# PROBIC/mSWEEP

Hardware: AMD Instinct MI355X
Metric: EM iters/sec + reads×groups cells/sec, 10M reads × 5k groups (higher is better)
Workload: dtype f64

## Files before the change

include/msweep_core.h:

```cpp
#ifndef MSWEEP_CORE_H
#define MSWEEP_CORE_H

#include <stddef.h>
#include <stdint.h>

#ifdef __cplusplus
extern "C" {
#endif

typedef struct msw_core *msw_handle;

enum { MSW_ALGO_RCG = 0, MSW_ALGO_EM = 1 };
enum { MSW_PREC_DOUBLE = 0, MSW_PREC_FLOAT = 1 };

int msw_core_create(int device, msw_handle *out);
void msw_core_destroy(msw_handle h);
const char *msw_last_error(msw_handle h);
const char *msw_core_version(void);


int msw_core_set_dense_logl(msw_handle h, const double *L, size_t n_groups, size_t n_ecs,
                            size_t ld);

int msw_core_set_csr(msw_handle h, const uint64_t *rowptr, const uint32_t *grp,
// ... 7 lines not shown
                              const uint64_t *ec_counts, double q, double e,
                              double zero_inflation, size_t min_hits,
                              size_t *n_groups_out, uint8_t *mask_out, double *logc_out);

int msw_core_get_dense_logl(msw_handle h, double *L_out, size_t ld);
int msw_core_layout_hash(msw_handle h, uint64_t *hash_out);
int msw_core_shape(msw_handle h, size_t *n_groups, size_t *n_ecs, size_t *nnz);
typedef struct msw_layout_info {
  int32_t record_bytes;
  int32_t index_records;
  int32_t groups_in_lds;
  int32_t table_in_lds;
  int32_t passB_mode;
  uint32_t slot_entries;
  uint32_t slot_entries_in_lds;
  uint32_t n_slices, n_long_ecs;
  uint64_t rows;
  uint64_t rows_from_memory;
  uint32_t slices_by_lanes[7];
  uint32_t max_rows;
  int32_t bank_scheduled;
  int32_t passB_reg_cells;
  uint64_t rows_over_8;
} msw_layout_info;
int msw_core_layout_info(msw_handle h, msw_layout_info *out);
int msw_core_set_pack_schedule(msw_handle h, int enabled);

enum { MSW_OPT_CHECK_EVERY = 0, MSW_OPT_INIT_BOUND = 1, MSW_OPT_EM_PRIOR = 2, MSW_OPT_EM_STOP = 3 };
int msw_core_set_option(msw_handle h, int option, double value);
int msw_core_get_option(msw_handle h, int option, double *value);

int msw_core_solve(msw_handle h, const double *logc, const double *alpha0, double tol,
                   size_t max_iters, int algo, int prec, double *theta_out,
                   size_t *iters_out, double *bound_out);

int msw_core_prepare(msw_handle h, const double *logc, const double *alpha0);
int msw_core_run(msw_handle h, double tol, size_t max_iters, int algo, int prec,
                 double *theta_out, size_t *iters_out, double *bound_out);

int msw_core_gamma(msw_handle h, double *gamma_out, size_t ld);

int msw_core_gamma_block(msw_handle h, size_t ec_begin, size_t ec_end, double *gamma_out, size_t ld);

int msw_core_bin_reads(msw_handle h, const uint64_t *ec_rptr, const uint32_t *ec_reads, size_t n_ecs,
                       const uint32_t *targets, const double *thresholds, size_t n_targets, uint64_t *bin_ptr,
                       uint32_t *reads_out, double *log_thr_out);
// ... 108 lines not shown
```

msweep_amd/core.py:

```python
import ctypes as C
import os

import numpy as np

_HERE = os.path.dirname(os.path.abspath(__file__))
LIB_PATH = os.environ.get("MSWEEP_CORE_LIB") or os.path.join(_HERE, "libmsweep_core.so")

ALGO_RCG, ALGO_EM = 0, 1
PREC_DOUBLE, PREC_FLOAT = 0, 1
TEXT_PROBS, TEXT_LOGL, TEXT_BITSEQ = 0, 1, 2
OPT_CHECK_EVERY, OPT_INIT_BOUND, OPT_EM_PRIOR, OPT_EM_STOP = 0, 1, 2, 3
_OPTS = {"check_every": OPT_CHECK_EVERY, "init_bound": OPT_INIT_BOUND, "em_prior": OPT_EM_PRIOR, "em_stop": OPT_EM_STOP}

EXPORTS = [
    "msw_core_create", "msw_core_destroy", "msw_last_error", "msw_core_version",
    "msw_core_set_dense_logl", "msw_core_set_csr", "msw_core_build_likelihood",
    "msw_core_get_dense_logl", "msw_core_layout_hash", "msw_core_shape", "msw_alignment_read",
    "msw_alignment_shape", "msw_alignment_export", "msw_alignment_view", "msw_alignment_destroy", "msw_alignment_last_error",
    "msw_alignment_read_device", "msw_core_build_likelihood_aln", "msw_core_trim", "msw_alignment_on_device", "msw_core_solve", "msw_core_prepare", "msw_core_run",
    "msw_core_gamma",
    "msw_core_trace", "msw_core_set_trace_theta", "msw_core_bootstrap",
    "msw_core_resample_counts", "msw_core_set_profiling", "msw_core_last_timing",
    "msw_core_set_fixed_iters", "msw_core_hbm_stream_rates", "msw_comm_unique_id", "msw_comm_create_rccl", "msw_comm_create_local",
    "msw_comm_destroy", "msw_core_set_comm", "msw_comm_last_error", "msw_core_bootstrap_dist",
# ... 2 lines not shown
    "msw_core_set_option", "msw_core_get_option", "msw_core_bin_reads", "msw_core_bin_reads_aln",
    "msw_core_text_block", "msw_core_format_g6", "msw_core_last_text_timing",
    "msw_core_gzip_begin", "msw_core_text_block_gzip", "msw_core_gzip_append", "msw_core_gzip_end", "msw_core_last_gzip_timing",
]


class MswError(RuntimeError):
    """Non-zero return from the C ABI (mirrors the std::runtime_error the C++ shim throws)."""


class Timing(C.Structure):
    _fields_ = [("solve_ms", C.c_double), ("passA_ms", C.c_double), ("passB_ms", C.c_double),
                ("passA_launches", C.c_uint64), ("passB_launches", C.c_uint64), ("iters", C.c_uint64),
                ("bytes_passA", C.c_uint64), ("bytes_passB", C.c_uint64), ("collective_ms", C.c_double),
                ("collectives", C.c_uint64), ("em_float_kernels", C.c_uint64)]


class LayoutInfo(C.Structure):
    _fields_ = [("record_bytes", C.c_int32), ("index_records", C.c_int32), ("groups_in_lds", C.c_int32),
                ("table_in_lds", C.c_int32), ("passB_mode", C.c_int32), ("slot_entries", C.c_uint32),
                ("slot_entries_in_lds", C.c_uint32), ("n_slices", C.c_uint32), ("n_long_ecs", C.c_uint32),
                ("rows", C.c_uint64), ("rows_from_memory", C.c_uint64), ("slices_by_lanes", C.c_uint32 * 7),
                ("max_rows", C.c_uint32), ("bank_scheduled", C.c_int32), ("passB_reg_cells", C.c_int32),
                ("rows_over_8", C.c_uint64)]


class BootstrapTiming(C.Structure):
    _fields_ = [("table_ms", C.c_double), ("solve_ms", C.c_double), ("gather_ms", C.c_double),
                ("replicates", C.c_uint64), ("iterations", C.c_uint64), ("table_reused", C.c_uint64)]


_lib = None


def source_hash():
    import hashlib
    csrc = os.path.join(_HERE, "csrc")
    h = hashlib.sha256()
    files = sorted(os.path.join(csrc, f) for f in os.listdir(csrc) if f.endswith((".hip", ".hpp", ".inc", ".h")))
    for f in files + [os.path.join(os.path.dirname(_HERE), "include", "msweep_core.h")]:
        h.update(os.path.basename(f).encode() + b"\0")
        h.update(open(f, "rb").read())
    return h.hexdigest()[:16]


def _check_fresh(L):
    if os.environ.get("MSWEEP_CORE_LIB"):
# ... 615 lines not shown
```

msweep_amd/csrc/common.hpp:

```cpp
#pragma once
#include <hip/hip_runtime.h>

#include <cstdint>
#include <cstdio>
#include <stdexcept>
#include <string>
#include <vector>

namespace msw {

constexpr int kWave = 64;
#ifndef MSW_PASS_THREADS_A
#define MSW_PASS_THREADS_A 1024
#endif
#ifndef MSW_PASS_THREADS_B
#define MSW_PASS_THREADS_B 768
#endif
#ifndef MSW_PASS_THREADS_B8
#define MSW_PASS_THREADS_B8 1024
#endif
constexpr int kPassThreads = MSW_PASS_THREADS_A;
constexpr int kPassThreadsB = MSW_PASS_THREADS_B;
constexpr int kPassThreadsB8 = MSW_PASS_THREADS_B8;
constexpr int kMaxTrace = 4096;
constexpr int kRedfinParts = 5;
constexpr int kRedfinGroups = 16;
#ifndef MSW_REDFIN_THREADS
#define MSW_REDFIN_THREADS 512
#endif
constexpr int kRedfinThreads = MSW_REDFIN_THREADS;
constexpr int kRedfinSlots = kRedfinThreads / kRedfinGroups;
#ifndef MSW_FX
#define MSW_FX 1
#endif
constexpr bool kFx = MSW_FX != 0;

struct HipError : std::runtime_error {
  using std::runtime_error::runtime_error;
};

#define MSW_HIP(expr)                                                                      \
  do {                                                                                     \
    hipError_t _e = (expr);                                                                \
    if (_e != hipSuccess) {                                                                \
      char _b[512];                                                                        \
      snprintf(_b, sizeof _b, "%s failed: %s (%s:%d)", #expr, hipGetErrorString(_e),       \
// ... 72 lines not shown
```

msweep_amd/csrc/host_likelihood.inc:

```
namespace {

void sell_from_device(msw_core *h, const uint32_t *d_rowptr, const uint32_t *d_grp, const uint32_t *d_idx,
                      const double *cell_val = nullptr);
bool compress_dense(msw_core *h, const double *Lm, size_t ld, const double *stage, size_t G, size_t E, bool force);

void reset_likelihood(msw_core *h) {
  Resident &L = h->lik;
  static_cast<LikShape &>(L) = LikShape{};
  h->solver.have_solution = false;
  h->solver.prepared = false;
  h->iperm.release();
  L.long_row = multilane() ? kLongRow : kLongRowOneLane;
  if (const char *lr = getenv("MSWEEP_LONG_ROW"))
    L.long_row = (uint32_t)std::min(std::max(atoi(lr), 16), (int)L.long_row);
}

constexpr uint8_t kRGroup[64] = {0, 0, 0, 0, 1, 1, 1, 1, 1, 1, 1, 1, 0, 0, 0, 0, 1, 1, 1, 1, 0, 0,
                                 0, 0, 0, 0, 0, 0, 1, 1, 1, 1, 2, 2, 2, 2, 3, 3, 3, 3, 3, 3, 3, 3,
                                 2, 2, 2, 2, 3, 3, 3, 3, 2, 2, 2, 2, 2, 2, 2, 2, 3, 3, 3, 3};

constexpr uint8_t kRPos[64] = {0, 1, 2,  3,  0,  1,  2,  3,  4,  5,  6,  7,  4,  5,  6,  7,  8,  9,  10, 11, 8, 9,
                               10, 11, 12, 13, 14, 15, 12, 13, 14, 15, 0,  1,  2,  3,  0,  1,  2,  3,  4,  5, 6, 7,
                               4,  5,  6,  7,  8,  9,  10, 11, 8,  9,  10, 11, 12, 13, 14, 15, 12, 13, 14, 15};

// ... 50 lines not shown

void finish_sell(msw_core *h) {
  Resident &L = h->lik;
  const uint32_t wg_for_slices = (L.nslices + (kPassThreads / 64) - 1) / (kPassThreads / 64);
  L.nblk = (int)std::max<uint32_t>(1, std::min<uint32_t>(std::max(wg_for_slices, L.n_long), (uint32_t)h->n_cu));
  L.nblk_dense = 0;
  L.flavor = 0;
  L.packed_scheduled = h->pack_schedule;
  L.rows_over8 = 0;
  L.passB_rc8 = false;
  if (L.nslices && L.enc == kEncNarrow && L.cls.s0[kSliceClasses - 1] == 0) {
    DevBuf<unsigned long long> d_over;
    d_over.alloc(1);
    d_over.zero(h->stream);
    hipLaunchKernelGGL(k_rows_over, dim3(std::min<uint32_t>((L.nslices + 255) / 256, (uint32_t)h->n_cu * 8)), dim3(256), 0,
                       h->stream, L.slice_off.p, L.nslices, 8u, d_over.p);
    unsigned long long over = 0;
    MSW_HIP(hipMemcpyAsync(&over, d_over.p, sizeof over, hipMemcpyDeviceToHost, h->stream));
    MSW_HIP(hipStreamSynchronize(h->stream));
    L.rows_over8 = over;
    L.passB_rc8 = 20 * over <= L.nslots / 64;
    if (const char *e = getenv("MSWEEP_PASSB_RC")) L.passB_rc8 = atoi(e) == 8;
  }
  alloc_solve_state(L, h->solver);
  MSW_HIP(hipStreamSynchronize(h->stream));
}

template <class RP>
void upload_sell(msw_core *h, const RP *rowptr, const uint32_t *cell_grp, const uint32_t *cell_idx) {
  Resident &L = h->lik;
  const uint32_t E = L.E, G = L.G, n_lut = L.n_lut;
  const uint64_t nnz_all = rowptr[E];
  std::vector<uint64_t> freq(std::max<uint32_t>(n_lut, 1), 0);
  for (uint64_t k = 0; k < nnz_all; ++k) ++freq[cell_idx[k]];
  const SlotPlan sp = plan_slot_area(h, freq);
  const std::vector<uint32_t> &canon = sp.canon, &hot_rank = sp.hot_rank;
  const uint32_t rep_base = sp.rep_base;
  const std::vector<uint32_t> used = {sp.sentinel_slot};
  const bool wide = L.wide(), hybrid = L.hybrid();
  const int rw = wide ? 2 : 1;
  const RecDec dec = L.dec;
  const uint32_t n_hot = L.n_tab_lds;
  auto entry_of = [&](int lane, uint32_t idx) -> uint32_t {
    const uint32_t j = hot_rank[idx];
    if (lane < 0 || j == UINT32_MAX) return canon[idx];
    return rep_base + (j >> 1) * 16 + 2 * (kRPos[lane] >> 1) + (j & 1);
// ... 459 lines not shown
```

msweep_amd/csrc/msweep_core.hip:

```cpp
#include "../../include/msweep_core.h"

#include <algorithm>
#include <array>
#include <cmath>
#include <chrono>
#include <cstring>
#include <limits>
#include <memory>
#include <string>
#include <thread>
#include <unordered_map>
#include <vector>

#include <zlib.h>

#include <rocprim/device/device_radix_sort.hpp>
#include <rocprim/device/device_scan.hpp>
#include <rocprim/iterator/counting_iterator.hpp>
#include <rocprim/iterator/transform_iterator.hpp>

#include "kernels.hpp"
#include "pack_kernels.hpp"
#include "compress_kernels.hpp"
#include "comm.hpp"
// ... 13 lines not shown

namespace {
thread_local std::string g_create_error;
constexpr size_t kLdsMax = 160 * 1024;
constexpr int kIterBatch = 16;
}


struct LikShape {
  int flavor = -1;
  uint32_t G = 0, E = 0, n_lut = 0, nslices = 0, n_long = 0;
  uint64_t nnz = 0, nslots = 0;
  int enc = kEncNarrow;
  bool glds = true, tlds = true;
  int gmodeB = 1;
  RecDec dec = {};
  uint32_t n_area = 0;
  uint32_t n_tab_lds = 0;
  SliceClasses cls = {};
  bool packed_scheduled = false;
  uint32_t long_row = kLongRow;
  uint64_t rows_over8 = 0;
  bool passB_rc8 = false;
  double logzi = 0.0;
  int nblk = 0;
  int nblk_dense = 0;
  int nreg = 0;
  bool have_logc_res = false;
};

struct Resident : LikShape {
  DevBuf<uint32_t> rec, slice_off, long_ptr, rec_long, perm;
  DevBuf<uint8_t> slice_hot;
  DevBuf<uint32_t> area_slot;
  DevBuf<double> lut_area;
  DevBuf<double> lut, Lt;
  DevBuf<double> trange;
  DevBuf<double> logc_res;
  bool wide() const { return enc == kEncWide; }
  bool hybrid() const { return enc == kEncIndex; }
  int n_tab_inline() const { return flavor == 0 && n_area <= (uint32_t)kTabInline ? (int)n_area : 0; }
  int npart_rows() const { return flavor == 0 ? nblk : (nreg >= 32 ? 4 * nblk_dense : nblk_dense); }
  uint32_t guard_cap() const {
    static_assert(kPassThreads / 64 <= 16 && kPassThreadsB / 64 <= 16, "guard_cap / guard_bits assume <= 16 wavefronts per workgroup");
    const uint32_t nb0 = (uint32_t)std::max(nblk, 1);
    return 64u * ((nslices + nb0 - 1) / nb0 + 16u) + (n_long + nb0 - 1) / nb0 + 16u;
// ... 227 lines not shown
  S.n_tab_lds = L.n_tab_lds;
  S.slice_hot = L.slice_hot.p;
  S.lut_area = L.lut_area.p;
  S.cls = L.cls;
  return S;
}
GuardDev guard_view(const Resident &L, const Solver &s) {
  return GuardDev{s.guard_list.p, s.guard_bits.p, s.guard_tail.p, L.lut_area.p, s.guard_err.p, s.guard_visits.p, L.guard_cap(),
                  L.guard_words()};
}

int passB_mode(const Resident &L, bool glds, uint32_t n_tab, bool index) {
  const uint32_t G = L.G;
  if (glds) {
    if (pass_lds_bytes(1, n_tab, G, false, index) > kLdsMax) return -1;
    if (8ull * (G + kSentinels) <= kAccFixed && pass_lds_bytes(2, n_tab, G, false, index) <= kLdsMax) return 2;
    return 1;
  }
  if (pass_lds_bytes(0, n_tab, G, false, index) > kLdsMax) return -1;
  if (getenv("MSWEEP_GLOBAL_ATOMICS")) return 0;
  if (pass_lds_bytes(3, n_tab, G, false, index) <= kLdsMax) return 3;
  if (pass_lds_bytes(4, n_tab, G, false, index) <= kLdsMax) return 4;
  return 0;
}

bool multilane() {
  const char *e = getenv("MSWEEP_MULTILANE");
  return !(e && atoi(e) == 0);
}
SliceClasses make_slice_classes(const uint32_t *n) {
  SliceClasses C = {};
  for (int c = 0; c < kSliceClasses; ++c) {
    const uint32_t per = 64u >> (kMaxLgm - c);
    C.p0[c + 1] = C.p0[c] + n[c];
    C.s0[c + 1] = C.s0[c] + (n[c] + per - 1) / per;
  }
  return C;
}

void choose_lds_mode(Resident &L) {
  const bool opts[4][2] = {{true, true}, {true, false}, {false, true}, {false, false}};
  const char *force = getenv("MSWEEP_FORCE_LDS");
  for (auto &o : opts) {
    if (force && strlen(force) == 2 && (o[0] != (force[0] == '1') || o[1] != (force[1] == '1'))) continue;
    const uint32_t n_tab = o[1] ? L.n_area : 0u;
    const int gmB = passB_mode(L, o[0], n_tab, false);
// ... 132 lines not shown
void launch_passA_t(const Resident &L, Solver &s) {
  const size_t lds = pass_lds_bytes(GL ? 1 : 0, L.n_tab_lds, L.G, true, ENC == kEncIndex);
  const bool ml = L.cls.s0[kSliceClasses - 1] > 0;
  auto k = ml ? k_passA<ENC, GL, TL, true> : k_passA<ENC, GL, TL, false>;
  prepare_sweep(k, lds, s.lds_attr[0][(ml ? 40 : 0) + ENC * 4 + (GL ? 2 : 0) + (TL ? 1 : 0)]);
  hipLaunchKernelGGL(k, dim3(L.nblk), dim3(pass_threads_A<ENC>()), lds, s.stream, s.sc.p, sell_view(L, s),
                     s.ew.p, s.tabA.p, s.partA.p, s.partR.p, (int)((L.G + kRedfinGroups - 1) / kRedfinGroups),
                     guard_view(L, s));
}
template <int ENC, int GM, bool TL>
void launch_passB_t(const Resident &L, Solver &s) {
  const size_t lds = pass_lds_bytes(GM, L.n_tab_lds, L.G, false, ENC == kEncIndex);
  const bool ml = L.cls.s0[kSliceClasses - 1] > 0;
  if constexpr (ENC == kEncNarrow) {
    if (L.passB_rc8 && !ml) {
      auto k8 = k_passB<ENC, GM, TL, false, 8>;
      prepare_sweep(k8, lds, s.lds_attr[2][2 * GM + (TL ? 1 : 0)]);
      const auto rg_of = [&](uint32_t g0) {
        return GM == 4 ? RangeB{g0, std::min<uint32_t>(kRangeGroups, L.G - g0), g0 == 0 ? 1 : 0} : RangeB{0, 0, 1};
      };
      for (uint32_t g0 = 0; g0 < (GM == 4 ? L.G : 1u); g0 += kRangeGroups)
        hipLaunchKernelGGL(k8, dim3(L.nblk), dim3(pass_threads_B<ENC, 8>()), lds, s.stream, s.sc.p, sell_view(L, s), s.e.p,
                           s.tabB.p, s.partAcc.p, s.partS.p, s.Acc.p, rg_of(g0), guard_view(L, s));
      return;
    }
  }
  auto k = ml ? k_passB<ENC, GM, TL, true> : k_passB<ENC, GM, TL, false>;
  prepare_sweep(k, lds, s.lds_attr[1][(ml ? 40 : 0) + ENC * 10 + 2 * GM + (TL ? 1 : 0)]);
  if (GM == 4) {
    for (uint32_t g0 = 0; g0 < L.G; g0 += kRangeGroups)
      hipLaunchKernelGGL(k, dim3(L.nblk), dim3(pass_threads_B<ENC>()), lds, s.stream, s.sc.p, sell_view(L, s), s.e.p,
                         s.tabB.p, s.partAcc.p, s.partS.p, s.Acc.p,
                         RangeB{g0, std::min<uint32_t>(kRangeGroups, L.G - g0), g0 == 0 ? 1 : 0}, guard_view(L, s));
    return;
  }
  hipLaunchKernelGGL(k, dim3(L.nblk), dim3(pass_threads_B<ENC>()), lds, s.stream, s.sc.p, sell_view(L, s), s.e.p,
                     s.tabB.p, s.partAcc.p, s.partS.p, s.Acc.p, RangeB{0, 0, 1}, guard_view(L, s));
}

#define MSW_DISPATCH3(fn, ...)                                                       \
  do {                                                                               \
    const int key = L.enc * 4 + (L.glds ? 2 : 0) + (L.tlds ? 1 : 0);              \
    switch (key) {                                                                   \
      case 0: fn<kEncNarrow, false, false>(__VA_ARGS__); break;                      \
      case 1: fn<kEncNarrow, false, true>(__VA_ARGS__); break;                       \
      case 2: fn<kEncNarrow, true, false>(__VA_ARGS__); break;                       \
// ... 572 lines not shown
  });
  if (rc != 0 && h) g_aln_error = msw_last_error(h);
  return rc;
}

int msw_core_layout_info(msw_handle h, msw_layout_info *out) {
  return guarded(h, [&] {
    if (!out) throw Fail("null out");
    const Resident &L = h->lik;
    if (L.flavor != 0) throw Fail("msw_core_layout_info: no CSR-of-ECs likelihood resident");
    msw_layout_info li = {};
    li.record_bytes = L.enc == kEncValue ? 12 : (L.wide() ? 8 : 4);
    li.index_records = L.hybrid() ? 1 : 0;
    li.groups_in_lds = L.glds ? 1 : 0;
    li.table_in_lds = L.tlds ? 1 : 0;
    li.passB_mode = L.gmodeB;
    li.slot_entries = L.n_area;
    li.slot_entries_in_lds = L.n_tab_lds;
    li.n_slices = L.nslices;
    li.n_long_ecs = L.n_long;
    li.bank_scheduled = L.packed_scheduled ? 1 : 0;
    li.passB_reg_cells = L.passB_rc8 ? 8 : kRegCells;
    li.rows_over_8 = L.rows_over8;
    std::vector<uint32_t> off((size_t)L.nslices + 1);
    MSW_HIP(hipMemcpy(off.data(), L.slice_off.p, off.size() * sizeof(uint32_t), hipMemcpyDeviceToHost));
    li.rows = off[L.nslices];
    for (int c = 0; c < kSliceClasses; ++c) li.slices_by_lanes[c] = L.cls.s0[c + 1] - L.cls.s0[c];
    for (uint32_t s2 = 0; s2 < L.nslices; ++s2) li.max_rows = std::max(li.max_rows, off[s2 + 1] - off[s2]);
    if (L.hybrid()) {
      std::vector<uint8_t> hot(std::max<uint32_t>(L.nslices, 1));
      MSW_HIP(hipMemcpy(hot.data(), L.slice_hot.p, hot.size(), hipMemcpyDeviceToHost));
      for (uint32_t s2 = 0; s2 < L.nslices; ++s2) li.rows_from_memory += (off[s2 + 1] - off[s2]) - hot[s2];
    } else if (!L.tlds && L.enc != kEncValue) {
      li.rows_from_memory = li.rows;
    }
    *out = li;
  });
}

int msw_core_layout_hash(msw_handle h, uint64_t *hash_out) {
  return guarded(h, [&] {
    if (!hash_out) throw Fail("null out");
    *hash_out = layout_hash(h->lik);
  });
}

// ... 437 lines not shown
```

msweep_amd/csrc/sell.hpp:

```cpp
#pragma once
#include "common.hpp"

namespace msw {

constexpr uint32_t kSentinels = 64;

#ifndef MSW_REG_CELLS
#define MSW_REG_CELLS 16
#endif
constexpr int kRowsPerLane = MSW_REG_CELLS;
static_assert(kRowsPerLane == 16 || kRowsPerLane == 12 || kRowsPerLane == 8, "slices of at most 16, 12 or 8 rows");
constexpr int kSliceClasses = 7;
constexpr uint32_t kMaxLgm = kSliceClasses - 1;
struct SliceClasses {
  uint32_t s0[kSliceClasses + 1], p0[kSliceClasses + 1];
};
__host__ __device__ inline int slice_class_of(uint32_t len, bool multilane) {
  if (!multilane) return kSliceClasses - 1;
  uint32_t lgm = 0;
  while (lgm < kMaxLgm && len > ((uint32_t)kRowsPerLane << lgm)) ++lgm;
  return (int)(kMaxLgm - lgm);
}
struct SliceGeo {
  uint32_t lgm, ec0, nec;
// ... 233 lines not shown
  return n_tab_lds ? ((16u * n_tab_lds + 255u) & ~255u) : 0u;
}
constexpr uint32_t kGeoStride = 66 * 8;
constexpr uint32_t kAccFixed = 65528;
__host__ __device__ inline uint32_t pass_acc_off(int gmode, uint32_t G) {
  return gmode >= 3 ? 0u : (gmode == 2 ? kAccFixed : 8u * (G + kSentinels));
}
constexpr uint32_t kRangeGroups = 16384;
struct RangeB {
  uint32_t g0, n;
  int first;
};
__host__ __device__ inline size_t pass_scratch_off(int gmode, uint32_t n_tab_lds, uint32_t G, bool passA, bool index) {
  const size_t bhi = sell_bhi(n_tab_lds), Gp = (size_t)G + kSentinels;
  if (gmode == 0 || (passA && gmode >= 3)) return bhi;
  if (passA) return (index ? bhi : 2 * bhi) + 16 * Gp;
  if (gmode == 4) return bhi + 8 * (size_t)kRangeGroups;
  return bhi + pass_acc_off(gmode, G) + 8 * Gp;
}
constexpr size_t kPassTailBytes = 32 * sizeof(double) + 16 * kGeoStride;
__host__ __device__ inline size_t pass_lds_bytes(int gmode, uint32_t n_tab_lds, uint32_t G, bool passA, bool index) {
  return pass_scratch_off(gmode, n_tab_lds, G, passA, index) + kPassTailBytes;
}

}
```

msweep_amd/csrc/sweep_kernels.hpp:

```cpp
#pragma once
#include <type_traits>

#include "device_util.hpp"
#include "sell.hpp"

namespace msw {

constexpr int kRegCells = kRowsPerLane;
#ifndef MSW_LONG_STEP
#define MSW_LONG_STEP 8
#endif
constexpr int kLongStep = MSW_LONG_STEP;
#ifndef MSW_REVERSE_B
#define MSW_REVERSE_B true
#endif
#ifndef MSW_B_KEEPN
#define MSW_B_KEEPN MSW_REG_CELLS
#endif
#ifndef MSW_PASSA_BATCH
#define MSW_PASSA_BATCH 4
#endif
#ifdef MSW_NO_PRIME
constexpr bool kPrimeFirstSlice = false;
#else
// ... 30 lines not shown
#endif
}
__device__ __forceinline__ double ec_div(double c, double z) {
#if MSW_FAST_DIV
  const double r = ec_rcp(z);
  const double q = c * r;
#if MSW_DIV_CORRECT
  return fma(fma(-z, q, c), r, q);
#else
  return q;
#endif
#else
  return c / z;
#endif
}

__device__ __forceinline__ uint32_t uniform(uint32_t v) { return __builtin_amdgcn_readfirstlane(v); }
__device__ __forceinline__ double uniform_d(double v) {
  const uint32_t lo = __builtin_amdgcn_readfirstlane(__double2loint(v));
  const uint32_t hi = __builtin_amdgcn_readfirstlane(__double2hiint(v));
  return __hiloint2double((int)hi, (int)lo);
}

template <int ENC, int RC = kRegCells>
struct SliceBuf {
  typename Rec<ENC>::T r[RC];
  typename Rec<ENC>::T rc[ENC == kEncIndex ? kColdRows : 1];
  uint32_t sl, o, len, nhot;
  uint32_t lgm, nec;
  uint32_t c8;
};

template <int ENC, int RC>
__device__ __forceinline__ void load_slice(const uint32_t *rec, size_t base, uint32_t len,
                                           typename Rec<ENC>::T (&r)[RC], typename Rec<ENC>::T nullr) {
#pragma unroll
  for (int k = 0; k < RC; k += 2) {
    if ((uint32_t)k < len) {
      r[k] = Rec<ENC>::load(rec, base + (size_t)k * 64);
      if constexpr (odd_slices(ENC)) {
        r[k + 1] = nullr;
        if ((uint32_t)k + 1 < len) r[k + 1] = Rec<ENC>::load(rec, base + (size_t)(k + 1) * 64);
      } else {
        r[k + 1] = Rec<ENC>::load(rec, base + (size_t)(k + 1) * 64);
      }
    }
// ... 8 lines not shown
#pragma unroll
    for (int j = 0; j < kColdRows; ++j)
      if ((uint32_t)j < ncold) rc[j] = rec[base + (size_t)(nhot + j) * 64];
  } else {
    load_slice<kEncIndex>(rec, base, len, r, nullr);
  }
}

template <int ENC>
__device__ __forceinline__ typename Rec<ENC>::T null_record(uint32_t g, const RecDec &d, double tnull) {
  if constexpr (ENC == kEncValue) return ValRec{8u * g, tnull};
  else return Rec<ENC>::make(g, 0u, d);
}
#ifndef MSW_VAL_THREADS
#define MSW_VAL_THREADS 512
#endif
#ifndef MSW_HYB_THREADS_A
#define MSW_HYB_THREADS_A MSW_PASS_THREADS_A
#endif
template <int ENC>
constexpr int pass_threads_A() {
  return ENC == kEncValue ? MSW_VAL_THREADS : (ENC == kEncIndex ? MSW_HYB_THREADS_A : kPassThreads);
}
template <int ENC, int RC = kRegCells>
constexpr int pass_threads_B() { return ENC == kEncValue ? MSW_VAL_THREADS : (RC < kRegCells ? kPassThreadsB8 : kPassThreadsB); }

__device__ __forceinline__ void wait_vm0() { __builtin_amdgcn_s_waitcnt(0x0F70); }

#ifdef MSW_EXPERIMENT_NOSTREAM
#define MSW_REC_ROW(o) ((o) & 1023u)
#else
#define MSW_REC_ROW(o) (o)
#endif
template <int ENC, bool REVERSE, int RC = kRegCells>
struct SliceStream {
  const SellDev &S;
  uint32_t s_first, nw, n_mine, lane;
  uint32_t geo;
  typename Rec<ENC>::T nullr = {};
  typename Rec<ENC>::T nullr_hot = {};
  uint2 pend = make_uint2(0, 0);
  __device__ __forceinline__ SliceStream(const SellDev &S_, uint32_t first, uint32_t nw_, uint32_t lane_,
                                         uint32_t geo_)
      : S(S_), s_first(first), nw(nw_), lane(lane_), geo(geo_) {
    n_mine = first < S.nslices ? (S.nslices - first + nw_ - 1) / nw_ : 0;
    gather_offs(0);
  }
  __device__ __forceinline__ uint32_t slice_at(uint32_t i) const {
// ... 381 lines not shown
            t1 = fma(q, ev.y, t1);
            t2 = fma(q * ev.y, ev.y, t2);
          }
        }
        atomicAnd(&bits[w0], 0u);
      }
      z = wave_sum(z), t1 = wave_sum(t1), t2 = wave_sum(t2);
      if (lane == 0) {
        if (z > 0.0) {
          const double S1 = t1 / z, S2 = t2 / z;
          nn += S2 - S1 * S1;
        } else {
          *GD.err = 1;
        }
      }
      __builtin_amdgcn_s_waitcnt(0);
    }
  }
  nn = block_sum_fixed1<NT / 64>(nn, sh);
  if (tid == 0) MSW_STAMP_MAX(sc->iter, 0, 7);
  if (tid == 0) partA[blockIdx.x] = nn;
}

template <int ENC, int GMODE, bool TLDS, bool ML, int RC = kRegCells>
__global__ __launch_bounds__((pass_threads_B<ENC, RC>())) void k_passB(const Scalars *sc, SellDev S, const double *e_g,
                                                       const double2 *tabB_g, double *partAcc,
                                                       double *partS, double *accGlobal, RangeB rg, GuardDev GD) {
  extern __shared__ __align__(16) unsigned char smem[];
  using R = Rec<ENC>;
  using RT = typename R::T;
  constexpr bool HYB = ENC == kEncIndex;
  constexpr bool VAL = ENC == kEncValue;
  constexpr int NT = pass_threads_B<ENC, RC>();
  static_assert(!((HYB || VAL) && TLDS), "index records go with the hybrid slot area, value records have no table");
  constexpr bool TL = TLDS || HYB;
  const RecDec D = rec_dec(S);
  const uint32_t n_tab = S.n_tab_lds;
  const int skip = sc->done;
  const int tid = threadIdx.x, lane = tid & 63;
  const uint32_t G = S.n_groups, Gp = G + kSentinels;
  const uint32_t bhi = S.bhi;
  constexpr bool GLDS = GMODE == 1 || GMODE == 2;
  constexpr bool ALDS = GMODE > 0;
  const uint32_t acc_off = pass_acc_off(GMODE, G);
  const uint32_t scratch_off = (uint32_t)pass_scratch_off(GMODE, n_tab, G, false, HYB);
  double *sh = reinterpret_cast<double *>(smem + scratch_off);
  SliceStream<ENC, MSW_REVERSE_B, RC> stream(S, uniform(blockIdx.x * (NT / 64) + (tid >> 6)),
                              gridDim.x * (NT / 64), (uint32_t)lane,
                              scratch_off + 256u + uniform(tid >> 6) * kGeoStride);
  [[maybe_unused]] const double vlogzi0 = uniform_d(sc->logzi);
  const uint32_t n_lanes = S.nslices * 64u;
  const RT null_rec = null_record<ENC>(G + (uint32_t)lane, D, vlogzi0);
  stream.nullr = null_rec;
  if constexpr (HYB) stream.nullr_hot = R::make_h(G + (uint32_t)lane, 0u, D);
  else stream.nullr_hot = null_rec;
  auto issue = [&](SliceBuf<ENC, RC> &sb) {
    const uint32_t q = sb.sl * 64 + lane;
// ... 54 lines not shown
    else if constexpr (GMODE == 3)
      __hip_atomic_fetch_add((LT *)(size_t)off, v, __ATOMIC_RELAXED, __HIP_MEMORY_SCOPE_WORKGROUP);
    else if constexpr (GMODE == 4) {
      const uint32_t d = off - bhi - 8u * rg.g0;
      if (d < 8u * rg.n)
        __hip_atomic_fetch_add((LT *)(size_t)(bhi + d), v, __ATOMIC_RELAXED, __HIP_MEMORY_SCOPE_WORKGROUP);
    }
    else
      atomicAdd(reinterpret_cast<V *>(acc_b + off), v);
  };
  auto addACC = [&](RT r, auto v) { addACCx(r, v, std::false_type{}); };
  auto addFXx = [&](RT r, double rs, double pk, auto HOT) { addACCx(r, fx_bits(rs, pk), HOT); };
  auto addFXwidex = [&](RT r, double rs, double pk, auto HOT) {
    const double q = rs * pk;
    const double vh = fma(q, 0x1p-32, kFxMagic);
    const double qh = vh - kFxMagic;
    const double ql = fma(-qh, 0x1p32, q);
    addACCx(r, (unsigned long long)(uint32_t)__double2loint(vh) << 32, HOT);
    addACCx(r, fx_bits(1.0, ql), HOT);
  };
  auto addFX = [&](RT r, double rs, double pk) { addFXx(r, rs, pk, std::false_type{}); };
  auto addFXwide = [&](RT r, double rs, double pk) { addFXwidex(r, rs, pk, std::false_type{}); };
  const double p0 = uniform_d(sc->p0), U = uniform_d(sc->U);
  const double zbase = p0 * U, hbase = p0 * uniform_d(sc->logzi) * U;
  const int fxe = (int)uniform((uint32_t)fx_expbits(sc->fx_shift));
  const double fxs = uniform_d(sc->fx_scale), fxb = ldexp(uniform_d(sc->xb), 1 - (int)uniform((uint32_t)sc->fx_shift));
  const double fxt1 = 0x1p51 / fxs, fxt2 = 0x1p51 / (fxs * fxb);
  const double gthr = fmax(zbase * kGuardRatio, 2.2250738585072014e-308);
  const uint32_t gcnt_off = scratch_off + 128u;
  typedef __attribute__((address_space(3))) uint32_t lds_u32_t;
  auto defer = [&](uint32_t p) {
    const uint32_t i = __hip_atomic_fetch_add((lds_u32_t *)(size_t)gcnt_off, 1u, __ATOMIC_RELAXED, __HIP_MEMORY_SCOPE_WORKGROUP);
    if (i < GD.cap) GD.list[(size_t)blockIdx.x * GD.cap + i] = p;
    else *GD.err = 2;
  };
  double s_clogZ = 0.0, s_rH = 0.0, s_W = 0.0;
  double lp_mant = 1.0;
  int lp_exp = 0;
  auto flush_logs = [&] {
    s_clogZ += log(lp_mant) + (double)lp_exp * 0.693147180559945309417232121458;
    lp_mant = 1.0;
    lp_exp = 0;
  };
  if (skip) return;
  if (tid == 0) *(lds_u32_t *)(size_t)gcnt_off = 0u;
  if (tid == 0 && blockIdx.x == 0) MSW_STAMP(sc->iter, 2, 0);
  __syncthreads();
  if (tid == 0 && blockIdx.x == 0) MSW_STAMP(sc->iter, 2, 1);

  auto process = [&](SliceBuf<ENC, RC> &sb) {
    const uint32_t o = sb.o, len = sb.len;
    double c = (double)sb.c8;
    if (__builtin_amdgcn_ballot_w64(sb.c8 == kC8Escape)) {
      if (sb.c8 == kC8Escape)
        c = S.cvec[S.n_long + (ML ? slice_geo(S.cls, sb.sl).ec0 + ((uint32_t)lane >> sb.lgm) : sb.sl * 64 + lane)];
      __builtin_amdgcn_s_waitcnt(0x0F70);
    }
    double zs = 0.0, hs = 0.0;
    constexpr int KEEPN = ENC == kEncWide ? 4 : (MSW_B_KEEPN < RC ? MSW_B_KEEPN : RC);
    double xv[KEEPN > 0 ? KEEPN : 1];
    auto fixed = [&](RT(&b)[RC], auto LEN, auto KEEP, auto ANY) {
      constexpr int L = decltype(LEN)::value;
      constexpr bool KP = decltype(KEEP)::value;
      constexpr int B = MSW_PASSB_BATCH;
#pragma unroll
      for (int k0 = 0; k0 < L; k0 += B) {
        double ev[B];
        double2 xt[B];
#pragma unroll
        for (int k = 0; k < B; ++k) {
          if (k0 + k < L) {
            if constexpr (decltype(ANY)::value) ev[k] = E_(b[k0 + k]), xt[k] = XTg_(b[k0 + k]);
            else ev[k] = Eh_(b[k0 + k]), xt[k] = XT_(b[k0 + k]);
          }
        }
#pragma unroll
        for (int k = 0; k < B; ++k) {
          if (k0 + k < L) {
            zs = fma(ev[k], xt[k].x, zs);
            hs = fma(ev[k], xt[k].y, hs);
            if constexpr (KP && KEEPN > 0)
              if (k0 + k < KEEPN) xv[k0 + k] = kFx ? fx_factor(ev[k], fxe) * xt[k].x : xt[k].x;
          }
        }
      }
    };
    auto cells = [&](RT(&b)[RC], uint32_t n, auto KEEP) {
// ... 100 lines not shown
                if constexpr (decltype(WIDE_ADD)::value) addFXwide(sb.rc[j], rs, xc[j]);
                else addFX(sb.rc[j], rs, xc[j]);
              } else {
                addACC(sb.rc[j], rs * xc[j]);
              }
            }
          }
        }
      };
      const uint32_t lgm = ML ? sb.lgm : 0u;
      bool spoke = true;
      if (ML && lgm != 0u) {
        zs = group_sum(zs, lgm);
        hs = group_sum(hs, lgm);
        spoke = ((uint32_t)lane & ((1u << lgm) - 1u)) == 0u;
      }
      if (c != 0.0 && !(zbase + zs >= gthr)) {
        if (spoke) defer(S.n_long + (ML ? slice_geo(S.cls, sb.sl).ec0 + ((uint32_t)lane >> lgm) : sb.sl * 64 + lane));
      } else if (c != 0.0) {
        const double Z = zbase + zs;
        const double rj = ec_div(c, Z);
        double rja = rj;
        if (ML && lgm != 0u) rja = spoke ? rj : 0.0;
        s_rH = fma(rja, hs, s_rH);
        s_W += rja;
        if constexpr (kFx) {
          const double rs = rj * fxs;
          if (fma(rj, zbase, c) < fxt1 && rj < fxt2) scatter_all(rs, std::false_type{});
          else scatter_all(rs, std::true_type{});
        } else {
          scatter_all(rj, std::false_type{});
        }
        __builtin_amdgcn_sched_barrier(0);
        if (sb.c8 <= 15u) {
          const int ez = __builtin_amdgcn_frexp_exp(Z);
          const double m = __builtin_amdgcn_frexp_mant(Z);
          double r;
          if (__builtin_amdgcn_ballot_w64(sb.c8 > 3u) == 0) {
            r = m;
            r *= sb.c8 >= 2u ? m : 1.0;
            r *= sb.c8 >= 3u ? m : 1.0;
          } else {
            const double m2 = m * m, m4 = m2 * m2, m8 = m4 * m4;
            r = (sb.c8 & 1u) ? m : 1.0;
            r *= (sb.c8 & 2u) ? m2 : 1.0;
            r *= (sb.c8 & 4u) ? m4 : 1.0;
            r *= (sb.c8 & 8u) ? m8 : 1.0;
          }
          int ezc = __mul24(ez, (int)sb.c8);
          if (ML && lgm != 0u && !spoke) r = 1.0, ezc = 0;
          lp_mant *= r;
          lp_exp += ezc;
        } else if (spoke) {
          s_clogZ += c * log(Z);
        }
      }
    } else {
      const size_t base = (size_t)o * 64 + lane;
      RT t[RC];
      uint32_t k0 = 0;
      for (; k0 + (uint32_t)RC <= len; k0 += RC) {
        load_slice<ENC>(S.rec, base + (size_t)k0 * 64, RC, t, null_rec);
        fixed(t, std::integral_constant<int, RC>{}, std::false_type{}, std::true_type{});
      }
      if (k0 < len) {
        const uint32_t n = len - k0;
        load_slice<ENC>(S.rec, base + (size_t)k0 * 64, n, t, null_rec);
        pairs_any(t, n);
      }
      if (c != 0.0 && !(zbase + zs >= gthr)) {
        defer(S.n_long + (ML ? slice_geo(S.cls, sb.sl).ec0 : sb.sl * 64) + lane);
      } else if (c != 0.0) {
        const double Z = zbase + zs;
        const double rj = ec_div(c, Z);
        s_clogZ += c * log(Z);
        s_rH = fma(rj, hs, s_rH);
        s_W += rj;
        const double rs = kFx ? rj * fxs : rj;
        const bool narrow = !kFx || (fma(rj, zbase, c) < fxt1 && rj < fxt2);
        for (k0 = 0; k0 < len; k0 += RC) {
          const uint32_t n = len - k0 < (uint32_t)RC ? len - k0 : (uint32_t)RC;
          load_slice<ENC>(S.rec, base + (size_t)k0 * 64, n, t, null_rec);
          if (narrow) scatter(t, n, rs, std::false_type{}, std::false_type{});
          else scatter(t, n, rs, std::false_type{}, std::true_type{});
        }
      }
    }
  };
  if constexpr (PRIME) stream.run(issue, process, flush_logs, &first);
  else stream.run(issue, process, flush_logs);
  {
    uint32_t r = stream.s_first, c0 = 0, c1 = 0;
    if (r < S.n_long) c0 = S.long_ptr[r], c1 = S.long_ptr[r + 1];
    auto load_long = [&](uint32_t kb, uint32_t k1, RT(&dst)[kLongStep]) {
#pragma unroll
      for (int u = 0; u < kLongStep; ++u) {
        dst[u] = null_rec;
        if (kb + 64u * u < k1 && kb + 64u * u + lane < k1) dst[u] = R::load(S.rec_long, kb + 64u * u + lane);
      }
    };
// ... 33 lines not shown
          }
        }
        kb += kLongStep * 64;
        if (kb >= c1) break;
        load_long(kb, c1, rc);
      }
      zs = wave_sum(zs);
      hs = wave_sum(hs);
      if (c != 0.0 && !(zbase + zs >= gthr)) {
        if (lane == 0) defer(r);
      } else if (c != 0.0) {
        const double Z = zbase + zs;
        const double rj = ec_div(c, Z);
        const uint32_t c8l = uniform((uint32_t)S.c8[r]);
        if (c8l <= 15u) {
          if (lane == 0) {
            int ez;
            const double m = frexp(Z, &ez);
            const double m2 = m * m, m4 = m2 * m2, m8 = m4 * m4;
            double pw = (c8l & 1u) ? m : 1.0;
            pw *= (c8l & 2u) ? m2 : 1.0;
            pw *= (c8l & 4u) ? m4 : 1.0;
            pw *= (c8l & 8u) ? m8 : 1.0;
            lp_mant *= pw;
            lp_exp += ez * (int)c8l;
          }
          if (++n_deferred == 32u) {
            flush_logs();
            n_deferred = 0;
          }
        } else if (lane == 0) {
          s_clogZ += c * log(Z);
        }
        if (lane == 0) {
          s_rH = fma(rj, hs, s_rH);
          s_W += rj;
        }
#pragma unroll
        for (int u = 0; u < kLongStep; ++u) rc[u] = first[u];
        const double rs = kFx ? rj * fxs : rj;
        const bool narrow = !kFx || (fma(rj, zbase, c) < fxt1 && rj < fxt2);
        for (uint32_t kb = c0;;) {
#pragma unroll
          for (int q = 0; q < kLongStep; q += 4) {
            if (kb + 64u * q < c1) {
              double xm[4];
              if (MSW_LONG_KEEP && kb == c0) {
#pragma unroll
                for (int u = 0; u < 4; ++u) xm[u] = pkf[q + u];
              } else {
#pragma unroll
                for (int u = 0; u < 4; ++u) xm[u] = kFx ? fx_factor(E_(rc[q + u]), fxe) * XMg_(rc[q + u]) : XMg_(rc[q + u]);
              }
#pragma unroll
              for (int u = 0; u < 4; ++u) {
                if constexpr (kFx) {
                  if (narrow) addFX(rc[q + u], rs, xm[u]);
                  else addFXwide(rc[q + u], rs, xm[u]);
                } else {
                  addACC(rc[q + u], rj * xm[u]);
// ... 29 lines not shown
      const uint32_t p = GD.list[(size_t)blockIdx.x * GD.cap + i];
      const double c = S.cvec[p];
      double z = 0.0, h = 0.0;
      wave_cells<ENC>(S, p, (uint32_t)lane, [&](uint32_t g, double T) {
        const double q = e_g[g] * exp(a * (T - tref));
        atomicOr(&bits[g >> 5], 1u << (g & 31));
        z += q;
        h = fma(q, T, h);
      });
      __builtin_amdgcn_s_waitcnt(0);
      double r0 = 0.0;
      for (uint32_t w0 = lane; w0 < GD.words; w0 += 64) {
        const uint32_t listed = atomicOr(&bits[w0], 0u);
        for (uint32_t b = 0; b < 32; ++b) {
          const uint32_t g = w0 * 32 + b;
          if (g < G && !((listed >> b) & 1u)) r0 += e_g[g];
        }
      }
      z = wave_sum(z), h = wave_sum(h), r0 = wave_sum(r0);
      const double Z = fma(p0, r0, z), H = fma(p0 * logzi, r0, h);
      if (Z > 0.0) {
        const double rj = c / Z;
        if (lane == 0) {
          s_clogZ += c * log(Z);
          s_rH += rj * H;
        }
        wave_cells<ENC>(S, p, (uint32_t)lane, [&](uint32_t g, double T) {
          add_share(g, e_g[g] * rj * exp(a * (T - tref)));
        });
        for (uint32_t w0 = lane; w0 < GD.words; w0 += 64) {
          const uint32_t listed = atomicAnd(&bits[w0], 0u);
          for (uint32_t b = 0; b < 32; ++b) {
            const uint32_t g = w0 * 32 + b;
            if (g < G && !((listed >> b) & 1u)) add_share(g, e_g[g] * (rj * p0));
          }
        }
      } else {
        if (lane == 0) *GD.err = 1;
        for (uint32_t w0 = lane; w0 < GD.words; w0 += 64) atomicAnd(&bits[w0], 0u);
      }
      __builtin_amdgcn_s_waitcnt(0);
    }
  }
  s_rH = fma(hbase, s_W, s_rH);
  {
    double t3[3] = {s_clogZ, s_rH, s_W};
    block_sum_n<3>(t3, sh + 32);
    if (tid == 0 && (GMODE != 4 || rg.first)) {
      partS[4 * blockIdx.x + 0] = t3[0];
      partS[4 * blockIdx.x + 1] = t3[1];
      partS[4 * blockIdx.x + 2] = t3[2];
      partS[4 * blockIdx.x + 3] = 0.0;
    }
  }
  if (tid == 0) MSW_STAMP_MAX(sc->iter, 2, 6);
  if (ALDS) {
    __syncthreads();
    const double *al = reinterpret_cast<const double *>(smem + bhi + acc_off);
    double *dst = partAcc + (size_t)blockIdx.x * G;
    if (GMODE == 4) {
      for (uint32_t g = tid; g < rg.n; g += NT) dst[rg.g0 + g] = al[g];
    } else {
      for (uint32_t g = tid; g < G; g += NT) dst[g] = al[g];
    }
  }
// ... 5 lines not shown
```

Measured before the change: 239200 billion.

## Park pass-B per-thread accumulators in LDS to run 16-wave blocks

```diff
diff --git a/include/msweep_core.h b/include/msweep_core.h
--- a/include/msweep_core.h
+++ b/include/msweep_core.h
@@ -53,6 +53,8 @@
   int32_t bank_scheduled;
   int32_t passB_reg_cells;
   uint64_t rows_over_8;
+  int32_t passB_waves;
+  uint32_t passB_lds_bytes;
 } msw_layout_info;
 int msw_core_layout_info(msw_handle h, msw_layout_info *out);
 int msw_core_set_pack_schedule(msw_handle h, int enabled);
diff --git a/msweep_amd/core.py b/msweep_amd/core.py
--- a/msweep_amd/core.py
+++ b/msweep_amd/core.py
@@ -48,7 +48,7 @@
                 ("slot_entries_in_lds", C.c_uint32), ("n_slices", C.c_uint32), ("n_long_ecs", C.c_uint32),
                 ("rows", C.c_uint64), ("rows_from_memory", C.c_uint64), ("slices_by_lanes", C.c_uint32 * 7),
                 ("max_rows", C.c_uint32), ("bank_scheduled", C.c_int32), ("passB_reg_cells", C.c_int32),
-                ("rows_over_8", C.c_uint64)]
+                ("rows_over_8", C.c_uint64), ("passB_waves", C.c_int32), ("passB_lds_bytes", C.c_uint32)]
 
 
 class BootstrapTiming(C.Structure):
diff --git a/msweep_amd/csrc/common.hpp b/msweep_amd/csrc/common.hpp
--- a/msweep_amd/csrc/common.hpp
+++ b/msweep_amd/csrc/common.hpp
@@ -22,6 +22,7 @@
 constexpr int kPassThreads = MSW_PASS_THREADS_A;
 constexpr int kPassThreadsB = MSW_PASS_THREADS_B;
 constexpr int kPassThreadsB8 = MSW_PASS_THREADS_B8;
+constexpr int kPassThreadsB16 = 1024;
 constexpr int kMaxTrace = 4096;
 constexpr int kRedfinParts = 5;
 constexpr int kRedfinGroups = 16;
diff --git a/msweep_amd/csrc/host_likelihood.inc b/msweep_amd/csrc/host_likelihood.inc
--- a/msweep_amd/csrc/host_likelihood.inc
+++ b/msweep_amd/csrc/host_likelihood.inc
@@ -96,6 +96,7 @@
     L.passB_rc8 = 20 * over <= L.nslots / 64;
     if (const char *e = getenv("MSWEEP_PASSB_RC")) L.passB_rc8 = atoi(e) == 8;
   }
+  L.passB_w16 = !L.passB_rc8 && passB_parked(L);
   alloc_solve_state(L, h->solver);
   MSW_HIP(hipStreamSynchronize(h->stream));
 }
diff --git a/msweep_amd/csrc/msweep_core.hip b/msweep_amd/csrc/msweep_core.hip
--- a/msweep_amd/csrc/msweep_core.hip
+++ b/msweep_amd/csrc/msweep_core.hip
@@ -59,6 +59,7 @@
   uint32_t long_row = kLongRow;
   uint64_t rows_over8 = 0;
   bool passB_rc8 = false;
+  bool passB_w16 = false;
   double logzi = 0.0;
   int nblk = 0;
   int nblk_dense = 0;
@@ -332,6 +333,19 @@
   if (pass_lds_bytes(3, n_tab, G, false, index) <= kLdsMax) return 3;
   if (pass_lds_bytes(4, n_tab, G, false, index) <= kLdsMax) return 4;
   return 0;
+}
+
+bool passB_parked(const Resident &L) {
+  if (L.enc != kEncNarrow || !L.tlds || (L.gmodeB != 1 && L.gmodeB != 2)) return false;
+  if (passB_lds_bytes(L.gmodeB, L.n_tab_lds, L.G, false, true) > kLdsMax) return false;
+  if (const char *e = getenv("MSWEEP_PASSB_WAVES")) return atoi(e) != 12;
+  return true;
+}
+int passB_waves(const Resident &L) {
+  if (L.enc == kEncValue) return pass_threads_B<kEncValue>() / 64;
+  const bool ml = L.cls.s0[kSliceClasses - 1] > 0;
+  if (L.enc == kEncNarrow && L.passB_rc8 && !ml) return pass_threads_B<kEncNarrow, 8>() / 64;
+  return (L.passB_w16 ? kPassThreadsB16 : kPassThreadsB) / 64;
 }
 
 bool multilane() {
@@ -510,6 +524,17 @@
       for (uint32_t g0 = 0; g0 < (GM == 4 ? L.G : 1u); g0 += kRangeGroups)
         hipLaunchKernelGGL(k8, dim3(L.nblk), dim3(pass_threads_B<ENC, 8>()), lds, s.stream, s.sc.p, sell_view(L, s), s.e.p,
                            s.tabB.p, s.partAcc.p, s.partS.p, s.Acc.p, rg_of(g0), guard_view(L, s));
+      return;
+    }
+  }
+  if constexpr (ENC == kEncNarrow && TL && (GM == 1 || GM == 2)) {
+    if (L.passB_w16) {
+      const size_t ldsp = passB_lds_bytes(GM, L.n_tab_lds, L.G, false, true);
+      auto kp = ml ? k_passB<ENC, GM, TL, true, kRegCells, true> : k_passB<ENC, GM, TL, false, kRegCells, true>;
+      prepare_sweep(kp, ldsp, s.lds_attr[2][40 + (ml ? 2 : 0) + (GM - 1)]);
+      hipLaunchKernelGGL(kp, dim3(L.nblk), dim3(pass_threads_B<ENC, kRegCells, true>()), ldsp, s.stream, s.sc.p,
+                         sell_view(L, s), s.e.p, s.tabB.p, s.partAcc.p, s.partS.p, s.Acc.p, RangeB{0, 0, 1},
+                         guard_view(L, s));
       return;
     }
   }
@@ -1128,6 +1153,8 @@
     li.bank_scheduled = L.packed_scheduled ? 1 : 0;
     li.passB_reg_cells = L.passB_rc8 ? 8 : kRegCells;
     li.rows_over_8 = L.rows_over8;
+    li.passB_waves = passB_waves(L);
+    li.passB_lds_bytes = (uint32_t)passB_lds_bytes(L.gmodeB, L.n_tab_lds, L.G, L.hybrid(), L.passB_w16);
     std::vector<uint32_t> off((size_t)L.nslices + 1);
     MSW_HIP(hipMemcpy(off.data(), L.slice_off.p, off.size() * sizeof(uint32_t), hipMemcpyDeviceToHost));
     li.rows = off[L.nslices];
diff --git a/msweep_amd/csrc/sell.hpp b/msweep_amd/csrc/sell.hpp
--- a/msweep_amd/csrc/sell.hpp
+++ b/msweep_amd/csrc/sell.hpp
@@ -279,5 +279,34 @@
 __host__ __device__ inline size_t pass_lds_bytes(int gmode, uint32_t n_tab_lds, uint32_t G, bool passA, bool index) {
   return pass_scratch_off(gmode, n_tab_lds, G, passA, index) + kPassTailBytes;
 }
-
-}
+constexpr uint32_t kParkPair = 16 * 64 * 16, kParkC = 16 * 64 * 8;
+struct ParkLayout {
+  uint32_t rw, lp, c;
+  size_t bytes;
+};
+__host__ __device__ inline ParkLayout passB_park_layout(int gmode, uint32_t n_tab_lds, uint32_t G, bool index) {
+  size_t tail = (pass_lds_bytes(gmode, n_tab_lds, G, false, index) + 15) & ~(size_t)15;
+  size_t hole = 0, hole_end = 0;
+  if (gmode == 2) {
+    const size_t bhi = sell_bhi(n_tab_lds);
+    hole = (bhi + 8 * ((size_t)G + kSentinels) + 15) & ~(size_t)15;
+    hole_end = bhi + kAccFixed;
+  }
+  auto place = [&](uint32_t n) -> uint32_t {
+    size_t &at = hole + n <= hole_end ? hole : tail;
+    const size_t o = at;
+    at += n;
+    return (uint32_t)o;
+  };
+  ParkLayout P;
+  P.rw = place(kParkPair);
+  P.lp = place(kParkPair);
+  P.c = place(kParkC);
+  P.bytes = tail;
+  return P;
+}
+__host__ __device__ inline size_t passB_lds_bytes(int gmode, uint32_t n_tab_lds, uint32_t G, bool index, bool parked) {
+  return parked ? passB_park_layout(gmode, n_tab_lds, G, index).bytes : pass_lds_bytes(gmode, n_tab_lds, G, false, index);
+}
+
+}
diff --git a/msweep_amd/csrc/sweep_kernels.hpp b/msweep_amd/csrc/sweep_kernels.hpp
--- a/msweep_amd/csrc/sweep_kernels.hpp
+++ b/msweep_amd/csrc/sweep_kernels.hpp
@@ -76,6 +76,12 @@
   return __hiloint2double((int)hi, (int)lo);
 }
 
+__device__ __forceinline__ double pin_uniform_d(double v) {
+  int lo = __double2loint(v), hi = __double2hiint(v);
+  asm volatile("" : "+v"(lo), "+v"(hi));
+  return __hiloint2double((int)uniform((uint32_t)hi), (int)uniform((uint32_t)lo));
+}
+
 template <int ENC, int RC = kRegCells>
 struct SliceBuf {
   typename Rec<ENC>::T r[RC];
@@ -130,8 +136,10 @@
 constexpr int pass_threads_A() {
   return ENC == kEncValue ? MSW_VAL_THREADS : (ENC == kEncIndex ? MSW_HYB_THREADS_A : kPassThreads);
 }
-template <int ENC, int RC = kRegCells>
-constexpr int pass_threads_B() { return ENC == kEncValue ? MSW_VAL_THREADS : (RC < kRegCells ? kPassThreadsB8 : kPassThreadsB); }
+template <int ENC, int RC = kRegCells, bool PARK = false>
+constexpr int pass_threads_B() {
+  return ENC == kEncValue ? MSW_VAL_THREADS : (RC < kRegCells ? kPassThreadsB8 : (PARK ? kPassThreadsB16 : kPassThreadsB));
+}
 
 __device__ __forceinline__ void wait_vm0() { __builtin_amdgcn_s_waitcnt(0x0F70); }
 
@@ -559,8 +567,8 @@
   if (tid == 0) partA[blockIdx.x] = nn;
 }
 
-template <int ENC, int GMODE, bool TLDS, bool ML, int RC = kRegCells>
-__global__ __launch_bounds__((pass_threads_B<ENC, RC>())) void k_passB(const Scalars *sc, SellDev S, const double *e_g,
+template <int ENC, int GMODE, bool TLDS, bool ML, int RC = kRegCells, bool PARK = false>
+__global__ __launch_bounds__((pass_threads_B<ENC, RC, PARK>())) void k_passB(const Scalars *sc, SellDev S, const double *e_g,
                                                        const double2 *tabB_g, double *partAcc,
                                                        double *partS, double *accGlobal, RangeB rg, GuardDev GD) {
   extern __shared__ __align__(16) unsigned char smem[];
@@ -568,8 +576,9 @@
   using RT = typename R::T;
   constexpr bool HYB = ENC == kEncIndex;
   constexpr bool VAL = ENC == kEncValue;
-  constexpr int NT = pass_threads_B<ENC, RC>();
+  constexpr int NT = pass_threads_B<ENC, RC, PARK>();
   static_assert(!((HYB || VAL) && TLDS), "index records go with the hybrid slot area, value records have no table");
+  static_assert(!PARK || (RC == kRegCells && !VAL), "the parked sums serve the 16-row kernel");
   constexpr bool TL = TLDS || HYB;
   const RecDec D = rec_dec(S);
   const uint32_t n_tab = S.n_tab_lds;
@@ -670,11 +679,15 @@
   auto addFX = [&](RT r, double rs, double pk) { addFXx(r, rs, pk, std::false_type{}); };
   auto addFXwide = [&](RT r, double rs, double pk) { addFXwidex(r, rs, pk, std::false_type{}); };
   const double p0 = uniform_d(sc->p0), U = uniform_d(sc->U);
-  const double zbase = p0 * U, hbase = p0 * uniform_d(sc->logzi) * U;
+  auto pin = [](double v) -> double {
+    if constexpr (PARK) return pin_uniform_d(v);
+    else return v;
+  };
+  const double zbase = pin(p0 * U), hbase = pin(p0 * uniform_d(sc->logzi) * U);
   const int fxe = (int)uniform((uint32_t)fx_expbits(sc->fx_shift));
   const double fxs = uniform_d(sc->fx_scale), fxb = ldexp(uniform_d(sc->xb), 1 - (int)uniform((uint32_t)sc->fx_shift));
-  const double fxt1 = 0x1p51 / fxs, fxt2 = 0x1p51 / (fxs * fxb);
-  const double gthr = fmax(zbase * kGuardRatio, 2.2250738585072014e-308);
+  const double fxt1 = pin(0x1p51 / fxs), fxt2 = pin(0x1p51 / (fxs * fxb));
+  const double gthr = pin(fmax(zbase * kGuardRatio, 2.2250738585072014e-308));
   const uint32_t gcnt_off = scratch_off + 128u;
   typedef __attribute__((address_space(3))) uint32_t lds_u32_t;
   auto defer = [&](uint32_t p) {
@@ -683,15 +696,56 @@
     else *GD.err = 2;
   };
   double s_clogZ = 0.0, s_rH = 0.0, s_W = 0.0;
-  double lp_mant = 1.0;
-  int lp_exp = 0;
+  [[maybe_unused]] double lp_mant = 1.0;
+  [[maybe_unused]] int lp_exp = 0;
+  typedef __attribute__((address_space(3))) v2d_t lds_d2_t;
+  [[maybe_unused]] const ParkLayout PL = PARK ? passB_park_layout(GMODE, n_tab, G, HYB) : ParkLayout{};
+  [[maybe_unused]] const uint32_t park = uniform(PL.rw) + (uint32_t)tid * 16u;
+  [[maybe_unused]] const uint32_t park_lp = uniform(PL.lp) + (uint32_t)tid * 16u;
+  [[maybe_unused]] auto park_c = [&]() -> uint32_t { return uniform(PL.c) + (uint32_t)tid * 8u; };
+  auto lp_pack = [](double m, int e) -> v2d_t { return v2d_t{m, __hiloint2double(0, e)}; };
+  auto add_rH_W = [&](double r, double h) {
+    if constexpr (PARK) {
+      v2d_t v = *(lds_d2_t *)(size_t)park;
+      v.x = fma(r, h, v.x);
+      v.y += r;
+      *(lds_d2_t *)(size_t)park = v;
+    } else {
+      s_rH = fma(r, h, s_rH);
+      s_W += r;
+    }
+  };
+  auto mul_lp = [&](double m, int e) {
+    if constexpr (PARK) {
+      const v2d_t v = *(lds_d2_t *)(size_t)(park_lp);
+      *(lds_d2_t *)(size_t)(park_lp) = lp_pack(v.x * m, __double2loint(v.y) + e);
+    } else {
+      lp_mant *= m;
+      lp_exp += e;
+    }
+  };
+  auto add_clogZ = [&](double v) {
+    if constexpr (PARK) *(lds_d_t *)(size_t)park_c() += v;
+    else s_clogZ += v;
+  };
   auto flush_logs = [&] {
-    s_clogZ += log(lp_mant) + (double)lp_exp * 0.693147180559945309417232121458;
-    lp_mant = 1.0;
-    lp_exp = 0;
+    if constexpr (PARK) {
+      const v2d_t v = *(lds_d2_t *)(size_t)(park_lp);
+      *(lds_d_t *)(size_t)park_c() += log(v.x) + (double)__double2loint(v.y) * 0.693147180559945309417232121458;
+      *(lds_d2_t *)(size_t)(park_lp) = lp_pack(1.0, 0);
+    } else {
+      s_clogZ += log(lp_mant) + (double)lp_exp * 0.693147180559945309417232121458;
+      lp_mant = 1.0;
+      lp_exp = 0;
+    }
   };
   if (skip) return;
   if (tid == 0) *(lds_u32_t *)(size_t)gcnt_off = 0u;
+  if constexpr (PARK) {
+    *(lds_d2_t *)(size_t)park = v2d_t{0.0, 0.0};
+    *(lds_d2_t *)(size_t)(park_lp) = lp_pack(1.0, 0);
+    *(lds_d_t *)(size_t)park_c() = 0.0;
+  }
   if (tid == 0 && blockIdx.x == 0) MSW_STAMP(sc->iter, 2, 0);
   __syncthreads();
   if (tid == 0 && blockIdx.x == 0) MSW_STAMP(sc->iter, 2, 1);
@@ -710,7 +764,7 @@
     auto fixed = [&](RT(&b)[RC], auto LEN, auto KEEP, auto ANY) {
       constexpr int L = decltype(LEN)::value;
       constexpr bool KP = decltype(KEEP)::value;
-      constexpr int B = MSW_PASSB_BATCH;
+      constexpr int B = PARK ? 2 : MSW_PASSB_BATCH;
 #pragma unroll
       for (int k0 = 0; k0 < L; k0 += B) {
         double ev[B];
@@ -857,8 +911,7 @@
         const double rj = ec_div(c, Z);
         double rja = rj;
         if (ML && lgm != 0u) rja = spoke ? rj : 0.0;
-        s_rH = fma(rja, hs, s_rH);
-        s_W += rja;
+        add_rH_W(rja, hs);
         if constexpr (kFx) {
           const double rs = rj * fxs;
           if (fma(rj, zbase, c) < fxt1 && rj < fxt2) scatter_all(rs, std::false_type{});
@@ -884,10 +937,9 @@
           }
           int ezc = __mul24(ez, (int)sb.c8);
           if (ML && lgm != 0u && !spoke) r = 1.0, ezc = 0;
-          lp_mant *= r;
-          lp_exp += ezc;
+          mul_lp(r, ezc);
         } else if (spoke) {
-          s_clogZ += c * log(Z);
+          add_clogZ(c * log(Z));
         }
       }
     } else {
@@ -908,9 +960,8 @@
       } else if (c != 0.0) {
         const double Z = zbase + zs;
         const double rj = ec_div(c, Z);
-        s_clogZ += c * log(Z);
-        s_rH = fma(rj, hs, s_rH);
-        s_W += rj;
+        add_clogZ(c * log(Z));
+        add_rH_W(rj, hs);
         const double rs = kFx ? rj * fxs : rj;
         const bool narrow = !kFx || (fma(rj, zbase, c) < fxt1 && rj < fxt2);
         for (k0 = 0; k0 < len; k0 += RC) {
@@ -990,20 +1041,16 @@
             pw *= (c8l & 2u) ? m2 : 1.0;
             pw *= (c8l & 4u) ? m4 : 1.0;
             pw *= (c8l & 8u) ? m8 : 1.0;
-            lp_mant *= pw;
-            lp_exp += ez * (int)c8l;
+            mul_lp(pw, ez * (int)c8l);
           }
           if (++n_deferred == 32u) {
             flush_logs();
             n_deferred = 0;
           }
         } else if (lane == 0) {
-          s_clogZ += c * log(Z);
-        }
-        if (lane == 0) {
-          s_rH = fma(rj, hs, s_rH);
-          s_W += rj;
-        }
+          add_clogZ(c * log(Z));
+        }
+        if (lane == 0) add_rH_W(rj, hs);
 #pragma unroll
         for (int u = 0; u < kLongStep; ++u) rc[u] = first[u];
         const double rs = kFx ? rj * fxs : rj;
@@ -1079,8 +1126,9 @@
       if (Z > 0.0) {
         const double rj = c / Z;
         if (lane == 0) {
-          s_clogZ += c * log(Z);
-          s_rH += rj * H;
+          add_clogZ(c * log(Z));
+          if constexpr (PARK) *(lds_d_t *)(size_t)park += rj * H;
+          else s_rH += rj * H;
         }
         wave_cells<ENC>(S, p, (uint32_t)lane, [&](uint32_t g, double T) {
           add_share(g, e_g[g] * rj * exp(a * (T - tref)));
@@ -1098,6 +1146,11 @@
       }
       __builtin_amdgcn_s_waitcnt(0);
     }
+  }
+  if constexpr (PARK) {
+    const v2d_t v = *(lds_d2_t *)(size_t)park;
+    s_rH = v.x, s_W = v.y;
+    s_clogZ = *(lds_d_t *)(size_t)park_c();
   }
   s_rH = fma(hbase, s_W, s_rH);
   {
```

New measurement: 236200 billion. 0.987x the previous value.
